# NUS-HPC-AI-Lab/VideoSys

Hardware: AMD Instinct MI355X
Metric: videos/min (Open-Sora 512x512x64f, 30 denoise steps, DiT denoising only) + sec/denoise-step (higher is better)
Workload: dtype bf16; 1 GPU; open-sora-v1.2 STDiT3-XL/2 512x512x64f, latent [4,19,64,64], CFG batch 2 = 38912 token rows, 300 text tokens, depth 28; steps_per_video=30, parallelism=dsp1

## Files before the change

__graft_entry__.py:

```python
from __future__ import annotations

import os
import subprocess
import sys

ROOT = os.path.dirname(os.path.abspath(__file__))
CSRC = os.path.join(ROOT, "videosys_amd", "csrc")
LIB = os.path.join(ROOT, "videosys_amd", "libvideosys_amd.so")
SOURCES = ["gemm_bf16.hip", "gemm2_bf16.hip", "conv_bf16.hip", "vae_ops.hip", "vae_sd3.hip", "vae_osp.hip", "t5_ops.hip", "clip_ops.hip", "rowwise.hip", "adaln_fold.hip", "attention.hip", "attention_w64.hip",
           "attention_t3.hip", "attention64.hip", "attention64_w64.hip", "attention_t64.hip", "attention96.hip", "attention96_img.hip", "p2p.hip", "capi.hip", "program.hip"]
LAB = os.environ.get("VSYS_LAB") == "1"
LAB_SOURCES = ["gemm3_bf16.hip", "gemm4_bf16.hip"]


def _hipcc():
    for c in (os.environ.get("HIPCC"), "/opt/rocm/bin/hipcc", "hipcc"):
        if c and (os.path.isabs(c) and os.path.exists(c) or not os.path.isabs(c)):
            return c
    return "hipcc"


HEADERS = [os.path.join(CSRC, "common.h"), os.path.join(CSRC, "vsys_internal.h"), os.path.join(CSRC, "flash72_w64_asm.inc"),
           os.path.join(CSRC, "program_ops.inc"), os.path.join(CSRC, "flash_w64.h"), os.path.join(CSRC, "attention96.h"), os.path.join(CSRC, "flash72_w64_map.inc"),
           os.path.join(ROOT, "include", "videosys_amd.h"),
           os.path.join(ROOT, "include", "videosys_amd_lab.h")]
FLAGS = ["--offload-arch=gfx950", "-O3", "-std=c++17", "-fPIC"]


def _is_lab(path):
    with open(path, "rb") as fh:
        return b"vsys_lab_flash_debug_buffer" in fh.read()


def _hipcc_id():
    try:
        return subprocess.run([_hipcc(), "--version"], capture_output=True, text=True, timeout=60).stdout.strip()[:400]
    except Exception:
        return "unknown"


def _digest(src, header_blob, flags, cc_id):
    import hashlib

    h = hashlib.sha256()
    h.update(cc_id.encode())
    h.update(" ".join(flags).encode())
    h.update(header_blob)
    with open(src, "rb") as fh:
        h.update(fh.read())
    return h.hexdigest()


ASM_OWNED = {"attention_w64.hip": 224, "attention64_w64.hip": 224}


def audit_asm_register_ownership(src: str, flags=None) -> None:
    import re
    import tempfile

    lo = ASM_OWNED[os.path.basename(src)]
    with tempfile.TemporaryDirectory() as d:
        out = os.path.join(d, "k.s")
        subprocess.run([_hipcc()] + (flags or FLAGS) + ["-S", "--cuda-device-only", "-o", out, src], check=True, capture_output=True,
                       cwd=CSRC)
        text = open(out).read().split("\n")
    inside, bad = False, []
    for ln in text:
        if "#ASMSTART" in ln:
            inside = True
        elif "#ASMEND" in ln:
            inside = False
        elif not inside and not ln.lstrip().startswith((".", ";")):
            code = ln.split(";")[0]
            regs = [int(m) for m in re.findall(r"\ba\[?(\d+)", code)]
            if any(r < lo for r in regs) or ("v_accvgpr" in code and not regs) or "scratch_" in code:
                bad.append(ln.strip())
    if bad:
        raise RuntimeError(f"{os.path.basename(src)}: compiler-generated code touches the asm statements' registers a[0:{lo - 1}] "
                           f"(or spills): {bad[:5]}")


def compile_library(out: str, lab: bool = False, objdir: str = None, force: bool = False) -> bool:
    import json
    from concurrent.futures import ThreadPoolExecutor

    import shutil

    if shutil.which(_hipcc()) is None and not os.path.isabs(_hipcc()) and os.path.exists(out) and not force:
        try:
            import json as _json

            with open(os.path.join(objdir or os.path.join(CSRC, "build", "lab" if lab else "ship"), "manifest.json")) as fh:
                man = _json.load(fh)
            blob = b""
            for h in HEADERS:
                with open(h, "rb") as fh:
                    blob += fh.read()
            flags = FLAGS + (["-DVSYS_LAB"] if lab else [])
            cc_id = man.get("compiler", "unknown")
            srcs = SOURCES + (LAB_SOURCES if lab else [])
            stale = [s_ for s_ in srcs if man.get("objects", {}).get(s_) != _digest(os.path.join(CSRC, s_), blob, flags, cc_id)]
        except Exception as e:
            stale = [f"(manifest unreadable: {e})"]
        if stale:
            raise RuntimeError(f"no hipcc on this box and the shipped {os.path.basename(out)} was not built from the current sources "
# ... 144 lines not shown
```

videosys_amd/csrc/rowwise.hip:

```cpp
#include "common.h"

#include <cstdlib>
#include "vsys_internal.h"

namespace vsys {
namespace {

template <int MAXV>
__global__ __launch_bounds__(256) void adaln_modulate_kernel(const bf16_t* __restrict__ x, const bf16_t* __restrict__ shift,
                                                             const bf16_t* __restrict__ scale, bf16_t* __restrict__ y,
                                                             int64_t rows, int C, int64_t rows_per_sample,
                                                             int64_t mod_stride, float eps) {
  const int lane = threadIdx.x & 63;
  const int64_t row = (int64_t)blockIdx.x * 4 + (threadIdx.x >> 6);
  if (row >= rows) return;
  const int nchunk = C >> 3;
  const bf16_t* xr = x + row * C;
  float v[MAXV][8];
  float s = 0.f;
#pragma unroll
  for (int i = 0; i < MAXV; ++i) {
    const int c = lane + 64 * i;
    if (c < nchunk) {
      uint4 u = *reinterpret_cast<const uint4*>(xr + c * 8);
      unpack8(u, v[i]);
#pragma unroll
      for (int e = 0; e < 8; ++e) s += v[i][e];
    }
  }
  const float mean = wave_sum(s) / (float)C;
  float q = 0.f;
#pragma unroll
  for (int i = 0; i < MAXV; ++i) {
    const int c = lane + 64 * i;
    if (c < nchunk) {
#pragma unroll
      for (int e = 0; e < 8; ++e) {
        float d = v[i][e] - mean;
        q += d * d;
      }
    }
  }
  const float rstd = rsqrtf(wave_sum(q) / (float)C + eps);
  const int64_t b = row / rows_per_sample;
  const bf16_t* sh = shift + b * mod_stride;
  const bf16_t* sc = scale + b * mod_stride;
  bf16_t* yr = y + row * C;
#pragma unroll
  for (int i = 0; i < MAXV; ++i) {
    const int c = lane + 64 * i;
    if (c < nchunk) {
      float a[8], m[8], o[8];
      unpack8(*reinterpret_cast<const uint4*>(sh + c * 8), a);
      unpack8(*reinterpret_cast<const uint4*>(sc + c * 8), m);
#pragma unroll
      for (int e = 0; e < 8; ++e) o[e] = (v[i][e] - mean) * rstd * (1.0f + m[e]) + a[e];
      *reinterpret_cast<uint4*>(yr + c * 8) = pack8(o);
    }
  }
}

template <int RPW>
__global__ __launch_bounds__(256) void adaln_modulate_rows_kernel(const bf16_t* __restrict__ x, const bf16_t* __restrict__ shift,
                                                                  const bf16_t* __restrict__ scale, bf16_t* __restrict__ y,
                                                                  int64_t rows, int C, int64_t rows_per_sample,
                                                                  int64_t mod_stride, float eps) {
  constexpr int MAXV = 3;
  const int lane = threadIdx.x & 63;
  const int64_t row0 = ((int64_t)blockIdx.x * 4 + (threadIdx.x >> 6)) * RPW;
  if (row0 >= rows) return;
  const int nchunk = C >> 3;
  uint4 u[RPW][MAXV];
#pragma unroll
  for (int r = 0; r < RPW; ++r) {
    const int64_t row = row0 + r < rows ? row0 + r : rows - 1;
#pragma unroll
    for (int i = 0; i < MAXV; ++i) {
      const int c = lane + 64 * i;
      u[r][i] = c < nchunk ? *reinterpret_cast<const uint4*>(x + row * C + c * 8) : make_uint4(0, 0, 0, 0);
    }
  }
  const int64_t b = row0 / rows_per_sample;
  uint4 ush[MAXV], usc[MAXV];
#pragma unroll
  for (int i = 0; i < MAXV; ++i) {
    const int c = lane + 64 * i;
    ush[i] = c < nchunk ? *reinterpret_cast<const uint4*>(shift + b * mod_stride + c * 8) : make_uint4(0, 0, 0, 0);
    usc[i] = c < nchunk ? *reinterpret_cast<const uint4*>(scale + b * mod_stride + c * 8) : make_uint4(0, 0, 0, 0);
  }
// ... 89 lines not shown
        float w[8], bb[8];
        unpack8(*reinterpret_cast<const uint4*>(ln_w + c * 8), w);
        unpack8(*reinterpret_cast<const uint4*>(ln_b + c * 8), bb);
#pragma unroll
        for (int e = 0; e < 8; ++e) o[e] = o[e] * w[e] + bb[e];
      }
      if (shift != nullptr) {
        float a[8], m[8];
        unpack8(*reinterpret_cast<const uint4*>(shift + b * mod_stride + alt + c * 8), a);
        unpack8(*reinterpret_cast<const uint4*>(scale + b * mod_stride + alt + c * 8), m);
#pragma unroll
        for (int e = 0; e < 8; ++e) o[e] = o[e] * (1.0f + m[e]) + a[e];
      }
      *reinterpret_cast<uint4*>(yr + c * 8) = pack8(o);
    }
  }
}

__global__ void gate_add_rows_kernel(bf16_t* __restrict__ x, const bf16_t* __restrict__ y, const bf16_t* __restrict__ gate,
                                     int64_t rows, int C8, int64_t rows_per_sample, int64_t gate_stride, int64_t seg_split,
                                     int64_t gate_alt) {
  const int64_t total = rows * C8;
  for (int64_t i = (int64_t)blockIdx.x * blockDim.x + threadIdx.x; i < total; i += (int64_t)gridDim.x * blockDim.x) {
    const int64_t r = i / C8;
    const int c = (int)(i - r * C8);
    const int64_t b = r / rows_per_sample;
    const int64_t alt = (seg_split > 0 && r - b * rows_per_sample < seg_split) ? gate_alt : 0;
    float a[8], v[8], g[8];
    unpack8(reinterpret_cast<const uint4*>(x)[i], a);
    unpack8(reinterpret_cast<const uint4*>(y)[i], v);
    unpack8(*reinterpret_cast<const uint4*>(gate + b * gate_stride + alt + c * 8), g);
#pragma unroll
    for (int k = 0; k < 8; ++k) a[k] += bf2f(f2bf(g[k] * v[k]));
    reinterpret_cast<uint4*>(x)[i] = pack8(a);
  }
}

__global__ void im2col_patch_kernel(const float* __restrict__ z, int Bz, bf16_t* __restrict__ out, int B, int F, int Cin, int H,
                                    int W, int p) {
  const int Hp = H / p, Wp = W / p, K = Cin * p * p;
  const int64_t total = (int64_t)B * F * Hp * Wp * K;
  for (int64_t i = (int64_t)blockIdx.x * blockDim.x + threadIdx.x; i < total; i += (int64_t)gridDim.x * blockDim.x) {
    const int k = (int)(i % K);
    const int64_t tok = i / K;
    const int wp = (int)(tok % Wp), hp = (int)((tok / Wp) % Hp), f = (int)((tok / ((int64_t)Wp * Hp)) % F);
    const int b = (int)(tok / ((int64_t)Wp * Hp * F));
    const int dx = k % p, dy = (k / p) % p, c = k / (p * p);
    out[i] = f2bf(z[((((int64_t)(b % Bz) * F + f) * Cin + c) * H + hp * p + dy) * W + wp * p + dx]);
  }
}

__global__ void unpatchify_cvx_kernel(const bf16_t* __restrict__ x, int64_t ldx, float* __restrict__ out, int B, int F, int Hp,
                                      int Wp, int Cout, int p) {
  const int H = Hp * p, W = Wp * p;
  const int64_t total = (int64_t)B * F * Cout * H * W;
  for (int64_t i = (int64_t)blockIdx.x * blockDim.x + threadIdx.x; i < total; i += (int64_t)gridDim.x * blockDim.x) {
    const int w = (int)(i % W), h = (int)((i / W) % H), c = (int)((i / ((int64_t)W * H)) % Cout);
    const int64_t bf = i / ((int64_t)W * H * Cout);
    const int64_t tok = (bf * Hp + h / p) * Wp + w / p;
    out[i] = bf2f(x[tok * ldx + (c * p + h % p) * p + w % p]);
  }
}

__global__ void mod_table_kernel(const bf16_t* __restrict__ table, const bf16_t* __restrict__ t_mlp, bf16_t* __restrict__ out,
                                 int nblk, int B, int C6) {
  const int64_t i = (int64_t)blockIdx.x * blockDim.x + threadIdx.x;
  const int64_t total = (int64_t)nblk * B * C6;
  if (i >= total) return;
  const int c = (int)(i % C6);
  const int b = (int)((i / C6) % B);
  const int k = (int)(i / ((int64_t)C6 * B));
  out[i] = f2bf(bf2f(table[(int64_t)k * C6 + c]) + bf2f(t_mlp[(int64_t)b * C6 + c]));
}

__global__ void timestep_embedding_kernel(const float* __restrict__ t, bf16_t* __restrict__ out, int B, int dim) {
  const int i = blockIdx.x * blockDim.x + threadIdx.x;
  const int half = dim / 2;
  if (i >= B * half) return;
  const int b = i / half, k = i - b * half;
  const float f = expf(-9.210340371976184f * (float)k / (float)half);
  const float a = t[b] * f;
  out[(int64_t)b * dim + k] = f2bf(cosf(a));
  out[(int64_t)b * dim + half + k] = f2bf(sinf(a));
}

__global__ __launch_bounds__(256) void patch_embed_kernel(const float* __restrict__ x, int Bz, const bf16_t* __restrict__ w,
                                                          const bf16_t* __restrict__ bias, const bf16_t* __restrict__ pos,
                                                          bf16_t* __restrict__ out, int B, int Cin, int T, int H, int W,
                                                          int ph, int pw, int C, int s0, int Sl) {
  const int Hp = (H + ph - 1) / ph, Wp = (W + pw - 1) / pw;
  const int S = Hp * Wp;
  const int cchunks = C >> 3;
  const int64_t total = (int64_t)B * T * Sl * cchunks;
  const int64_t i = (int64_t)blockIdx.x * blockDim.x + threadIdx.x;
  if (i >= total) return;
  const int cc = (int)(i % cchunks);
  const int64_t tok = i / cchunks;
  const int s = s0 + (int)(tok % Sl);
  const int t = (int)((tok / Sl) % T);
  const int b = (int)(tok / ((int64_t)Sl * T));
  const int bz = b % Bz;
  if (s >= S) {
    *reinterpret_cast<uint4*>(out + tok * C + cc * 8) = make_uint4(0, 0, 0, 0);
    return;
  }
  const int hp = s / Wp, wp = s - hp * Wp;
  float acc[8];
  {
    float bb[8];
    unpack8(*reinterpret_cast<const uint4*>(bias + cc * 8), bb);
#pragma unroll
    for (int e = 0; e < 8; ++e) acc[e] = bb[e];
  }
  const int K = Cin * ph * pw;
  if (K == 16) {
    float xin[16];
#pragma unroll
    for (int k = 0; k < 16; ++k) {
      const int ci = k >> 2, dy = (k >> 1) & 1, dx = k & 1;
      const int hh = hp * 2 + dy, ww = wp * 2 + dx;
      xin[k] = 0.f;
      if (ph == 2 && pw == 2 && hh < H && ww < W) xin[k] = bf2f(f2bf(x[((((int64_t)bz * Cin + ci) * T + t) * H + hh) * W + ww]));
    }
    if (ph == 2 && pw == 2) {
#pragma unroll
      for (int e = 0; e < 8; ++e) {
        const bf16_t* wr = w + (int64_t)(cc * 8 + e) * 16;
        float wa[8], wb[8];
        unpack8(*reinterpret_cast<const uint4*>(wr), wa);
        unpack8(*reinterpret_cast<const uint4*>(wr + 8), wb);
#pragma unroll
        for (int k = 0; k < 8; ++k) acc[e] += xin[k] * wa[k] + xin[k + 8] * wb[k];
      }
    }
  }
  if (!(K == 16 && ph == 2 && pw == 2)) {
    for (int ci = 0; ci < Cin; ++ci)
      for (int dy = 0; dy < ph; ++dy)
        for (int dx = 0; dx < pw; ++dx) {
          const int hh = hp * ph + dy, ww = wp * pw + dx;
          float xv = 0.f;
          if (hh < H && ww < W) xv = bf2f(f2bf(x[((((int64_t)bz * Cin + ci) * T + t) * H + hh) * W + ww]));
          const int k = (ci * ph + dy) * pw + dx;
#pragma unroll
          for (int e = 0; e < 8; ++e) acc[e] += xv * bf2f(w[(int64_t)(cc * 8 + e) * K + k]);
        }
  }
  float pp[8];
  unpack8(*reinterpret_cast<const uint4*>(pos + (int64_t)s * C + cc * 8), pp);
#pragma unroll
  for (int e = 0; e < 8; ++e) acc[e] = bf2f(f2bf(acc[e])) + pp[e];
  *reinterpret_cast<uint4*>(out + tok * C + cc * 8) = pack8(acc);
}

template <int MAXV>
__global__ __launch_bounds__(256) void final_layer_kernel(const bf16_t* __restrict__ x, const bf16_t* __restrict__ table,
                                                          const bf16_t* __restrict__ tvec, const bf16_t* __restrict__ w,
                                                          const bf16_t* __restrict__ bias, float* __restrict__ out,
                                                          int B, int T, int Hp, int Wp, int H, int W, int ph, int pw,
                                                          int Cout, int C, float eps, int Sl, float* __restrict__ tokens) {
  const int lane = threadIdx.x & 63;
  const int S = Sl;
  const int64_t rows = (int64_t)B * T * S;
  const int64_t row = (int64_t)blockIdx.x * 4 + (threadIdx.x >> 6);
  if (row >= rows) return;
  const int nchunk = C >> 3;
  const bf16_t* xr = x + row * C;
  float v[MAXV][8];
  float s = 0.f;
#pragma unroll
  for (int i = 0; i < MAXV; ++i) {
    const int c = lane + 64 * i;
    if (c < nchunk) {
      unpack8(*reinterpret_cast<const uint4*>(xr + c * 8), v[i]);
#pragma unroll
      for (int e = 0; e < 8; ++e) s += v[i][e];
    } else {
#pragma unroll
      for (int e = 0; e < 8; ++e) v[i][e] = 0.f;
    }
  }
  const float mean = wave_sum(s) / (float)C;
  float q = 0.f;
#pragma unroll
  for (int i = 0; i < MAXV; ++i) {
    const int c = lane + 64 * i;
    if (c < nchunk) {
#pragma unroll
      for (int e = 0; e < 8; ++e) {
        float d = v[i][e] - mean;
        q += d * d;
      }
    }
  }
  const float rstd = rsqrtf(wave_sum(q) / (float)C + eps);
  const int b = (int)(row / ((int64_t)T * S));
#pragma unroll
  for (int i = 0; i < MAXV; ++i) {
    const int c = lane + 64 * i;
    if (c < nchunk) {
      float sh[8], sc[8], tt[8];
      unpack8(*reinterpret_cast<const uint4*>(table + c * 8), sh);
      unpack8(*reinterpret_cast<const uint4*>(table + C + c * 8), sc);
      unpack8(*reinterpret_cast<const uint4*>(tvec + (int64_t)b * C + c * 8), tt);
#pragma unroll
      for (int e = 0; e < 8; ++e) {
        const float shift = bf2f(f2bf(sh[e] + tt[e])), scale = bf2f(f2bf(sc[e] + tt[e]));
        v[i][e] = bf2f(f2bf((v[i][e] - mean) * rstd * (1.0f + scale) + shift));
      }
    }
  }
  const int NOUT = ph * pw * Cout;
  const int64_t tok = row % ((int64_t)T * S);
  const int t = (int)(tok / S), sidx = (int)(tok % S);
  const int hp = sidx / Wp, wp = sidx - hp * Wp;
  for (int n = 0; n < NOUT; ++n) {
    const bf16_t* wr = w + (int64_t)n * C;
    float d = 0.f;
#pragma unroll
    for (int i = 0; i < MAXV; ++i) {
      const int c = lane + 64 * i;
      if (c < nchunk) {
        float ww[8];
        unpack8(*reinterpret_cast<const uint4*>(wr + c * 8), ww);
#pragma unroll
        for (int e = 0; e < 8; ++e) d += v[i][e] * ww[e];
      }
    }
    d = wave_sum(d);
    if (lane == 0) {
      d = bf2f(f2bf(d + bf2f(bias[n])));
      if (tokens != nullptr) {
        tokens[row * NOUT + n] = d;
        continue;
      }
      const int co = n % Cout;
      const int dx = (n / Cout) % pw, dy = n / (Cout * pw);
      const int hh = hp * ph + dy, ww2 = wp * pw + dx;
      if (hh < H && ww2 < W) out[((((int64_t)b * Cout + co) * T + t) * H + hh) * W + ww2] = d;
    }
  }
}

__global__ void unpatchify_tokens_kernel(const float* __restrict__ tok, float* __restrict__ out, int P, int B, int T, int Sl,
                                         int Hp, int Wp, int H, int W, int ph, int pw, int Cout) {
  const int NOUT = ph * pw * Cout;
  const int64_t total = (int64_t)B * Cout * T * H * W;
  const int64_t i = (int64_t)blockIdx.x * blockDim.x + threadIdx.x;
  if (i >= total) return;
  const int ww = (int)(i % W), hh = (int)((i / W) % H), t = (int)((i / ((int64_t)W * H)) % T);
  const int co = (int)((i / ((int64_t)W * H * T)) % Cout), b = (int)(i / ((int64_t)W * H * T * Cout));
  const int hp = hh / ph, dy = hh - hp * ph, wp = ww / pw, dx = ww - wp * pw;
  const int s = hp * Wp + wp;
  const int r = s / Sl, j = s - r * Sl;
  const int n = (dy * pw + dx) * Cout + co;
  out[i] = tok[((((int64_t)r * B + b) * T + t) * Sl + j) * NOUT + n];
}

__global__ void cfg_euler_kernel(float* __restrict__ z, const float* __restrict__ model_out, int Bz, int Cin, int Cout,
                                 int64_t thw, float guidance, float dt) {
  const int64_t i = (int64_t)blockIdx.x * blockDim.x + threadIdx.x;
  const int64_t total = (int64_t)Bz * Cin * thw;
  if (i >= total) return;
  const int64_t sp = i % thw;
  const int c = (int)((i / thw) % Cin);
  const int b = (int)(i / (thw * Cin));
  const float cond = model_out[((int64_t)b * Cout + c) * thw + sp];
  const float unc = model_out[((int64_t)(b + Bz) * Cout + c) * thw + sp];
  z[i] = z[i] + (unc + guidance * (cond - unc)) * dt;
}

__global__ void cfg_axpby_kernel(float* __restrict__ z, const float* __restrict__ model_out, int Bz, int Cin, int Cout,
                                 int64_t thw, float guidance, float c_z, float c_eps, int cond_first) {
  const int64_t i = (int64_t)blockIdx.x * blockDim.x + threadIdx.x;
  const int64_t total = (int64_t)Bz * Cin * thw;
  if (i >= total) return;
  const int64_t sp = i % thw;
  const int c = (int)((i / thw) % Cin);
  const int b = (int)(i / (thw * Cin));
  const float h0 = model_out[((int64_t)b * Cout + c) * thw + sp];
  const float h1 = model_out[((int64_t)(b + Bz) * Cout + c) * thw + sp];
  const float cond = cond_first ? h0 : h1, unc = cond_first ? h1 : h0;
  z[i] = c_z * z[i] + c_eps * (unc + guidance * (cond - unc));
}

__global__ void add_bcast_rows_kernel(bf16_t* __restrict__ x, const bf16_t* __restrict__ e, int64_t rows, int C8, int64_t group,
                                      int64_t period) {
  const int64_t total = rows * C8;
  for (int64_t i = (int64_t)blockIdx.x * blockDim.x + threadIdx.x; i < total; i += (int64_t)gridDim.x * blockDim.x) {
    const int64_t r = i / C8;
    const int c = (int)(i - r * C8);
    const int64_t er = (r / group) % period;
    float a[8], b[8];
    unpack8(reinterpret_cast<const uint4*>(x)[i], a);
    unpack8(reinterpret_cast<const uint4*>(e)[er * C8 + c], b);
#pragma unroll
    for (int k = 0; k < 8; ++k) a[k] += b[k];
    reinterpret_cast<uint4*>(x)[i] = pack8(a);
  }
}

__global__ void add_rows_kernel(bf16_t* __restrict__ x, const bf16_t* __restrict__ y, int64_t n8) {
  for (int64_t i = (int64_t)blockIdx.x * blockDim.x + threadIdx.x; i < n8; i += (int64_t)gridDim.x * blockDim.x) {
    float a[8], b[8];
    unpack8(reinterpret_cast<const uint4*>(x)[i], a);
    unpack8(reinterpret_cast<const uint4*>(y)[i], b);
#pragma unroll
    for (int e = 0; e < 8; ++e) a[e] += b[e];
    reinterpret_cast<uint4*>(x)[i] = pack8(a);
  }
}

__global__ void scale_add_rows_kernel(const bf16_t* __restrict__ a, int64_t lda, const bf16_t* __restrict__ b, int64_t ldb,
                                      bf16_t* __restrict__ out, int64_t ldo, int64_t rows, int C8, float scale) {
  const int64_t total = rows * C8;
  for (int64_t i = (int64_t)blockIdx.x * blockDim.x + threadIdx.x; i < total; i += (int64_t)gridDim.x * blockDim.x) {
    const int64_t r = i / C8;
    const int c = (int)(i - r * C8) * 8;
    float x[8], y[8];
    unpack8(*reinterpret_cast<const uint4*>(a + r * lda + c), x);
    unpack8(*reinterpret_cast<const uint4*>(b + r * ldb + c), y);
#pragma unroll
// ... 78 lines not shown
    hipLaunchKernelGGL(adaln_modulate_kernel<2>, dim3(grid), dim3(256), 0, stream, x, shift, scale, y, rows, C,
                       rows_per_sample, mod_stride, eps);
  else if (C <= 64 * 8 * 3)
    hipLaunchKernelGGL(adaln_modulate_kernel<3>, dim3(grid), dim3(256), 0, stream, x, shift, scale, y, rows, C,
                       rows_per_sample, mod_stride, eps);
  else
    hipLaunchKernelGGL(adaln_modulate_kernel<4>, dim3(grid), dim3(256), 0, stream, x, shift, scale, y, rows, C,
                       rows_per_sample, mod_stride, eps);
  return hipGetLastError() == hipSuccess ? 0 : VSYS_ERR_LAUNCH;
}

int launch_ln_modulate(const bf16_t* x, const bf16_t* ln_w, const bf16_t* ln_b, const bf16_t* shift, const bf16_t* scale,
                       bf16_t* y, int64_t rows, int C, int64_t rows_per_sample, int64_t mod_stride, int64_t seg_split,
                       int64_t mod_alt, float eps, hipStream_t stream) {
  if (rows <= 0) return 0;
  if (C % 8 != 0 || C > 64 * 8 * 6 || rows_per_sample <= 0 || (mod_stride % 8) || (mod_alt % 8)) return VSYS_ERR_SHAPE;
  if ((ln_w == nullptr) != (ln_b == nullptr) || (shift == nullptr) != (scale == nullptr)) return VSYS_ERR_ARG;
  const unsigned grid = (unsigned)((rows + 3) / 4);
#define VSYS_LNMOD(V)                                                                                                      \
  hipLaunchKernelGGL(ln_modulate_kernel<V>, dim3(grid), dim3(256), 0, stream, x, ln_w, ln_b, shift, scale, y, rows, C,       \
                     rows_per_sample, mod_stride, seg_split, mod_alt, eps)
  if (C <= 64 * 8 * 2) VSYS_LNMOD(2);
  else if (C <= 64 * 8 * 3) VSYS_LNMOD(3);
  else if (C <= 64 * 8 * 4) VSYS_LNMOD(4);
  else VSYS_LNMOD(6);
#undef VSYS_LNMOD
  return hipGetLastError() == hipSuccess ? 0 : VSYS_ERR_LAUNCH;
}

int launch_gate_add_rows(bf16_t* x, const bf16_t* y, const bf16_t* gate, int64_t rows, int C, int64_t rows_per_sample,
                         int64_t gate_stride, int64_t seg_split, int64_t gate_alt, hipStream_t stream) {
  if (rows <= 0) return 0;
  if (C % 8 || rows_per_sample <= 0 || (gate_stride % 8) || (gate_alt % 8)) return VSYS_ERR_SHAPE;
  int64_t grid = (rows * (C / 8) + 255) / 256;
  if (grid > 2048 * 4) grid = 2048 * 4;
  hipLaunchKernelGGL(gate_add_rows_kernel, dim3((unsigned)grid), dim3(256), 0, stream, x, y, gate, rows, C / 8, rows_per_sample,
                     gate_stride, seg_split, gate_alt);
  return hipGetLastError() == hipSuccess ? 0 : VSYS_ERR_LAUNCH;
}

int launch_im2col_patch(const float* z, int Bz, bf16_t* out, int B, int F, int Cin, int H, int W, int p, hipStream_t stream) {
  if (p <= 0 || H % p || W % p || Bz <= 0) return VSYS_ERR_SHAPE;
  const int64_t total = (int64_t)B * F * (H / p) * (W / p) * Cin * p * p;
  if (total <= 0) return 0;
  int64_t grid = (total + 255) / 256;
  if (grid > 2048 * 8) grid = 2048 * 8;
  hipLaunchKernelGGL(im2col_patch_kernel, dim3((unsigned)grid), dim3(256), 0, stream, z, Bz, out, B, F, Cin, H, W, p);
  return hipGetLastError() == hipSuccess ? 0 : VSYS_ERR_LAUNCH;
}

int launch_unpatchify_cvx(const bf16_t* x, int64_t ldx, float* out, int B, int F, int Hp, int Wp, int Cout, int p,
                          hipStream_t stream) {
  const int64_t total = (int64_t)B * F * Cout * Hp * p * Wp * p;
  if (total <= 0) return 0;
  int64_t grid = (total + 255) / 256;
  if (grid > 2048 * 8) grid = 2048 * 8;
  hipLaunchKernelGGL(unpatchify_cvx_kernel, dim3((unsigned)grid), dim3(256), 0, stream, x, ldx, out, B, F, Hp, Wp, Cout, p);
  return hipGetLastError() == hipSuccess ? 0 : VSYS_ERR_LAUNCH;
}

int launch_mod_table(const bf16_t* table, const bf16_t* t_mlp, bf16_t* out, int nblk, int B, int C6, hipStream_t stream) {
  const int64_t total = (int64_t)nblk * B * C6;
  if (total <= 0) return 0;
  hipLaunchKernelGGL(mod_table_kernel, dim3((unsigned)((total + 255) / 256)), dim3(256), 0, stream, table, t_mlp, out, nblk,
                     B, C6);
  return hipGetLastError() == hipSuccess ? 0 : VSYS_ERR_LAUNCH;
}

int launch_timestep_embedding(const float* t, bf16_t* out, int B, int dim, hipStream_t stream) {
  if (dim % 2) return VSYS_ERR_SHAPE;
  const int total = B * (dim / 2);
  if (total <= 0) return 0;
  hipLaunchKernelGGL(timestep_embedding_kernel, dim3((total + 127) / 128), dim3(128), 0, stream, t, out, B, dim);
  return hipGetLastError() == hipSuccess ? 0 : VSYS_ERR_LAUNCH;
}

int launch_patch_embed(const float* x, int Bz, const bf16_t* w, const bf16_t* bias, const bf16_t* pos, bf16_t* out, int B,
                       int Cin, int T, int H, int W, int ph, int pw, int C, int s0, int Sl, hipStream_t stream) {
  if (C % 8 || Bz <= 0 || s0 < 0) return VSYS_ERR_SHAPE;
  const int Hp = (H + ph - 1) / ph, Wp = (W + pw - 1) / pw;
  if (Sl < 0) Sl = Hp * Wp;
  const int64_t total = (int64_t)B * T * Sl * (C / 8);
  if (total <= 0) return 0;
  if ((total + 255) / 256 > 0x7fffffff) return VSYS_ERR_SHAPE;
  hipLaunchKernelGGL(patch_embed_kernel, dim3((unsigned)((total + 255) / 256)), dim3(256), 0, stream, x, Bz, w, bias, pos, out,
                     B, Cin, T, H, W, ph, pw, C, s0, Sl);
  return hipGetLastError() == hipSuccess ? 0 : VSYS_ERR_LAUNCH;
}

int launch_unpatchify_tokens(const float* tok, float* out, int P, int B, int T, int Sl, int Hp, int Wp, int H, int W, int ph,
                             int pw, int Cout, hipStream_t stream) {
  if (P <= 0 || Sl <= 0 || (int64_t)P * Sl < (int64_t)Hp * Wp) return VSYS_ERR_SHAPE;
  const int64_t total = (int64_t)B * Cout * T * H * W;
  if (total <= 0) return 0;
  if ((total + 255) / 256 > 0x7fffffff) return VSYS_ERR_SHAPE;
  hipLaunchKernelGGL(unpatchify_tokens_kernel, dim3((unsigned)((total + 255) / 256)), dim3(256), 0, stream, tok, out, P, B, T, Sl,
                     Hp, Wp, H, W, ph, pw, Cout);
  return hipGetLastError() == hipSuccess ? 0 : VSYS_ERR_LAUNCH;
}

int launch_final_layer(const bf16_t* x, const bf16_t* table, const bf16_t* tvec, const bf16_t* w, const bf16_t* bias,
                       float* out, int B, int T, int Hp, int Wp, int H, int W, int ph, int pw, int Cout, int C, float eps,
                       int Sl, float* tokens, hipStream_t stream) {
  if (C % 8 != 0 || C > 64 * 8 * 4) return VSYS_ERR_SHAPE;
  if (Sl < 0) Sl = Hp * Wp;
  if (tokens == nullptr && Sl != Hp * Wp) return VSYS_ERR_ARG;
  const int64_t rows = (int64_t)B * T * Sl;
  if (rows <= 0) return 0;
  const unsigned grid = (unsigned)((rows + 3) / 4);
  if (C <= 64 * 8 * 2)
    hipLaunchKernelGGL(final_layer_kernel<2>, dim3(grid), dim3(256), 0, stream, x, table, tvec, w, bias, out, B, T, Hp, Wp,
                       H, W, ph, pw, Cout, C, eps, Sl, tokens);
  else if (C <= 64 * 8 * 3)
    hipLaunchKernelGGL(final_layer_kernel<3>, dim3(grid), dim3(256), 0, stream, x, table, tvec, w, bias, out, B, T, Hp, Wp,
                       H, W, ph, pw, Cout, C, eps, Sl, tokens);
  else
    hipLaunchKernelGGL(final_layer_kernel<4>, dim3(grid), dim3(256), 0, stream, x, table, tvec, w, bias, out, B, T, Hp, Wp,
                       H, W, ph, pw, Cout, C, eps, Sl, tokens);
  return hipGetLastError() == hipSuccess ? 0 : VSYS_ERR_LAUNCH;
}

int launch_cfg_euler(float* z, const float* model_out, int Bz, int Cin, int Cout, int64_t thw, float guidance, float dt,
                     hipStream_t stream) {
  const int64_t total = (int64_t)Bz * Cin * thw;
  if (total <= 0) return 0;
  hipLaunchKernelGGL(cfg_euler_kernel, dim3((unsigned)((total + 255) / 256)), dim3(256), 0, stream, z, model_out, Bz, Cin,
                     Cout, thw, guidance, dt);
  return hipGetLastError() == hipSuccess ? 0 : VSYS_ERR_LAUNCH;
}

int launch_cfg_axpby(float* z, const float* model_out, int Bz, int Cin, int Cout, int64_t thw, float guidance, float c_z,
                     float c_eps, int cond_first, hipStream_t stream) {
  const int64_t total = (int64_t)Bz * Cin * thw;
  if (total <= 0) return 0;
  hipLaunchKernelGGL(cfg_axpby_kernel, dim3((unsigned)((total + 255) / 256)), dim3(256), 0, stream, z, model_out, Bz, Cin,
                     Cout, thw, guidance, c_z, c_eps, cond_first);
  return hipGetLastError() == hipSuccess ? 0 : VSYS_ERR_LAUNCH;
}

int launch_add_bcast_rows(bf16_t* x, const bf16_t* e, int64_t rows, int C, int64_t group, int64_t period, hipStream_t stream) {
  if (rows <= 0) return 0;
  if (C % 8 || group <= 0 || period <= 0) return VSYS_ERR_SHAPE;
  int64_t grid = (rows * (C / 8) + 255) / 256;
  if (grid > 2048 * 4) grid = 2048 * 4;
  hipLaunchKernelGGL(add_bcast_rows_kernel, dim3((unsigned)grid), dim3(256), 0, stream, x, e, rows, C / 8, group, period);
  return hipGetLastError() == hipSuccess ? 0 : VSYS_ERR_LAUNCH;
}

int launch_add_rows(bf16_t* x, const bf16_t* y, int64_t n, hipStream_t stream) {
  if (n <= 0) return 0;
  if (n % 8) return VSYS_ERR_SHAPE;
  const int64_t n8 = n / 8;
  int64_t grid = (n8 + 255) / 256;
  if (grid > 2048 * 4) grid = 2048 * 4;
  hipLaunchKernelGGL(add_rows_kernel, dim3((unsigned)grid), dim3(256), 0, stream, x, y, n8);
  return hipGetLastError() == hipSuccess ? 0 : VSYS_ERR_LAUNCH;
}

int launch_scale_add_rows(const bf16_t* a, int64_t lda, const bf16_t* b, int64_t ldb, bf16_t* out, int64_t ldo, int64_t rows, int C,
                          float scale, hipStream_t stream) {
  if (rows < 0 || C < 0) return VSYS_ERR_SHAPE;
  if (rows == 0 || C == 0) return 0;
  if (C % 8 || lda < C || ldb < C || ldo < C) return VSYS_ERR_SHAPE;
  if ((lda % 8) || (ldb % 8) || (ldo % 8) || reinterpret_cast<uintptr_t>(a) % 16 || reinterpret_cast<uintptr_t>(b) % 16 ||
      reinterpret_cast<uintptr_t>(out) % 16)
    return VSYS_ERR_ALIGN;
  int64_t grid = (rows * (C / 8) + 255) / 256;
  if (grid > 2048 * 4) grid = 2048 * 4;
  hipLaunchKernelGGL(scale_add_rows_kernel, dim3((unsigned)grid), dim3(256), 0, stream, a, lda, b, ldb, out, ldo, rows, C / 8, scale);
  return hipGetLastError() == hipSuccess ? 0 : VSYS_ERR_LAUNCH;
}

int launch_copy_4d(const bf16_t* src, bf16_t* dst, int n0, int n1, int n2, int C, int64_t ss0, int64_t ss1, int64_t ss2,
                   int64_t ds0, int64_t ds1, int64_t ds2, int n1_valid, int n2_valid, hipStream_t stream) {
  if (C % 8) return VSYS_ERR_SHAPE;
  const int64_t total = (int64_t)n0 * n1 * n2 * (C / 8);
  if (total <= 0) return 0;
  int64_t grid = (total + 255) / 256;
  if (grid > 2048 * 4) grid = 2048 * 4;
  hipLaunchKernelGGL(copy_4d_kernel, dim3((unsigned)grid), dim3(256), 0, stream, src, dst, n0, n1, n2, C, ss0, ss1, ss2, ds0,
                     ds1, ds2, n1_valid, n2_valid);
  return hipGetLastError() == hipSuccess ? 0 : VSYS_ERR_LAUNCH;
}

}
```

Before: 21.32 videos/min.

## Add persistent tiled kernels for patch embedding and final layer

```diff
diff --git a/__graft_entry__.py b/__graft_entry__.py
--- a/__graft_entry__.py
+++ b/__graft_entry__.py
@@ -20,7 +20,7 @@
     return "hipcc"
 
 
-HEADERS = [os.path.join(CSRC, "common.h"), os.path.join(CSRC, "vsys_internal.h"), os.path.join(CSRC, "flash72_w64_asm.inc"),
+HEADERS = [os.path.join(CSRC, "common.h"), os.path.join(CSRC, "vsys_internal.h"), os.path.join(CSRC, "rowwise_plan.h"), os.path.join(CSRC, "flash72_w64_asm.inc"),
            os.path.join(CSRC, "program_ops.inc"), os.path.join(CSRC, "flash_w64.h"), os.path.join(CSRC, "attention96.h"), os.path.join(CSRC, "flash72_w64_map.inc"),
            os.path.join(ROOT, "include", "videosys_amd.h"),
            os.path.join(ROOT, "include", "videosys_amd_lab.h")]
diff --git a/videosys_amd/csrc/rowwise.hip b/videosys_amd/csrc/rowwise.hip
--- a/videosys_amd/csrc/rowwise.hip
+++ b/videosys_amd/csrc/rowwise.hip
@@ -2,9 +2,15 @@
 
 #include <cstdlib>
 #include "vsys_internal.h"
+#include "rowwise_plan.h"
 
 namespace vsys {
 namespace {
+
+bool rowwise_edges_on() {
+  static const bool on = [] { const char* e = getenv("VSYS_ROWWISE_EDGES"); return !(e && e[0] == '0'); }();
+  return on;
+}
 
 template <int MAXV>
 __global__ __launch_bounds__(256) void adaln_modulate_kernel(const bf16_t* __restrict__ x, const bf16_t* __restrict__ shift,
@@ -260,6 +266,35 @@
   const float a = t[b] * f;
   out[(int64_t)b * dim + k] = f2bf(cosf(a));
   out[(int64_t)b * dim + half + k] = f2bf(sinf(a));
+}
+
+__device__ __forceinline__ void pe_bias_init(float (&acc)[8], const uint4& bias8) {
+  float bb[8];
+  unpack8(bias8, bb);
+#pragma unroll
+  for (int e = 0; e < 8; ++e) acc[e] = bb[e];
+}
+__device__ __forceinline__ void pe_load_weights(const bf16_t* __restrict__ w, int cc, float (&wa)[8][8], float (&wb)[8][8]) {
+#pragma unroll
+  for (int e = 0; e < 8; ++e) {
+    const bf16_t* wr = w + (int64_t)(cc * 8 + e) * 16;
+    unpack8(*reinterpret_cast<const uint4*>(wr), wa[e]);
+    unpack8(*reinterpret_cast<const uint4*>(wr + 8), wb[e]);
+  }
+}
+__device__ __forceinline__ void pe_conv16(float (&acc)[8], const float (&xin)[16], const float (&wa)[8][8], const float (&wb)[8][8]) {
+#pragma unroll
+  for (int e = 0; e < 8; ++e) {
+#pragma unroll
+    for (int k = 0; k < 8; ++k) acc[e] += xin[k] * wa[e][k] + xin[k + 8] * wb[e][k];
+  }
+}
+__device__ __forceinline__ uint4 pe_finish(float (&acc)[8], const uint4& pos8) {
+  float pp[8];
+  unpack8(pos8, pp);
+#pragma unroll
+  for (int e = 0; e < 8; ++e) acc[e] = bf2f(f2bf(acc[e])) + pp[e];
+  return pack8(acc);
 }
 
 __global__ __launch_bounds__(256) void patch_embed_kernel(const float* __restrict__ x, int Bz, const bf16_t* __restrict__ w,
@@ -284,12 +319,7 @@
   }
   const int hp = s / Wp, wp = s - hp * Wp;
   float acc[8];
-  {
-    float bb[8];
-    unpack8(*reinterpret_cast<const uint4*>(bias + cc * 8), bb);
-#pragma unroll
-    for (int e = 0; e < 8; ++e) acc[e] = bb[e];
-  }
+  pe_bias_init(acc, *reinterpret_cast<const uint4*>(bias + cc * 8));
   const int K = Cin * ph * pw;
   if (K == 16) {
     float xin[16];
@@ -301,15 +331,9 @@
       if (ph == 2 && pw == 2 && hh < H && ww < W) xin[k] = bf2f(f2bf(x[((((int64_t)bz * Cin + ci) * T + t) * H + hh) * W + ww]));
     }
     if (ph == 2 && pw == 2) {
-#pragma unroll
-      for (int e = 0; e < 8; ++e) {
-        const bf16_t* wr = w + (int64_t)(cc * 8 + e) * 16;
-        float wa[8], wb[8];
-        unpack8(*reinterpret_cast<const uint4*>(wr), wa);
-        unpack8(*reinterpret_cast<const uint4*>(wr + 8), wb);
-#pragma unroll
-        for (int k = 0; k < 8; ++k) acc[e] += xin[k] * wa[k] + xin[k + 8] * wb[k];
-      }
+      float wa[8][8], wb[8][8];
+      pe_load_weights(w, cc, wa, wb);
+      pe_conv16(acc, xin, wa, wb);
     }
   }
   if (!(K == 16 && ph == 2 && pw == 2)) {
@@ -324,12 +348,160 @@
           for (int e = 0; e < 8; ++e) acc[e] += xv * bf2f(w[(int64_t)(cc * 8 + e) * K + k]);
         }
   }
-  float pp[8];
-  unpack8(*reinterpret_cast<const uint4*>(pos + (int64_t)s * C + cc * 8), pp);
-#pragma unroll
-  for (int e = 0; e < 8; ++e) acc[e] = bf2f(f2bf(acc[e])) + pp[e];
-  *reinterpret_cast<uint4*>(out + tok * C + cc * 8) = pack8(acc);
-}
+  *reinterpret_cast<uint4*>(out + tok * C + cc * 8) = pe_finish(acc, *reinterpret_cast<const uint4*>(pos + (int64_t)s * C + cc * 8));
+}
+
+__global__ __launch_bounds__(PE_CHUNK_LANES* PE_TOKEN_LANES) void patch_embed_runs_kernel(
+    const float* __restrict__ x, int Bz, const bf16_t* __restrict__ w, const bf16_t* __restrict__ bias, const bf16_t* __restrict__ pos,
+    bf16_t* __restrict__ out, int B, int T, int H, int W, int C, int s0, int Sl, int runs_per_row, int run_len) {
+  constexpr int Cin = 4, NT = PE_CHUNK_LANES * PE_TOKEN_LANES;
+  __shared__ float xs[2 * Cin][2 * PE_RUN_TOKENS];
+  const int Hp = (H + 1) / 2, Wp = (W + 1) / 2;
+  const int cchunks = C >> 3;
+  const int tid = threadIdx.x;
+  const int tl = tid / PE_CHUNK_LANES;
+  const int cc = blockIdx.y * PE_CHUNK_LANES + (tid - tl * PE_CHUNK_LANES);
+  const bool active = cc < cchunks;
+  float wa[8][8], wb[8][8];
+  uint4 bias8 = make_uint4(0, 0, 0, 0);
+  if (active) {
+    pe_load_weights(w, cc, wa, wb);
+    bias8 = *reinterpret_cast<const uint4*>(bias + cc * 8);
+  }
+  const int hp0 = s0 / Wp, hp1 = (int)(((int64_t)s0 + Sl + Wp - 1) / Wp);
+  const int nhp = hp1 - hp0;
+  const int64_t nruns = (int64_t)B * T * nhp * runs_per_row;
+  for (int64_t run = blockIdx.x; run < nruns; run += gridDim.x) {
+    const int rw = (int)(run % runs_per_row);
+    int64_t r = run / runs_per_row;
+    const int hp = hp0 + (int)(r % nhp);
+    r /= nhp;
+    const int t = (int)(r % T), b = (int)(r / T);
+    const int wp0 = rw * run_len;
+    const int ntok = (Wp - wp0 < run_len ? Wp - wp0 : run_len);
+    if (hp < Hp) {
+      const int bz = b % Bz;
+      const int ncol = 2 * ntok;
+      for (int i = tid; i < 2 * Cin * ncol; i += NT) {
+        const int rr = i / ncol, col = i - rr * ncol;
+        const int hh = hp * 2 + (rr & 1), ww = wp0 * 2 + col;
+        float v = 0.f;
+        if (hh < H && ww < W) v = bf2f(f2bf(x[((((int64_t)bz * Cin + (rr >> 1)) * T + t) * H + hh) * W + ww]));
+        xs[rr][col] = v;
+      }
+    }
+    __syncthreads();
+    if (active) {
+      const int sb = hp * Wp + wp0;
+      auto load_pos = [&](int j) {
+        const int s = sb + j;
+        return (j < ntok && hp < Hp && s >= s0 && s - s0 < Sl) ? *reinterpret_cast<const uint4*>(pos + (int64_t)s * C + cc * 8)
+                                                              : make_uint4(0, 0, 0, 0);
+      };
+      uint4 p0 = load_pos(tl), p1 = load_pos(tl + PE_TOKEN_LANES);
+      for (int j = tl; j < ntok; j += PE_TOKEN_LANES) {
+        const uint4 pos8 = p0;
+        p0 = p1;
+        p1 = load_pos(j + 2 * PE_TOKEN_LANES);
+        const int s = sb + j;
+        if (s >= s0 && s - s0 < Sl) {
+          bf16_t* o = out + (((int64_t)b * T + t) * Sl + (s - s0)) * C + cc * 8;
+          if (hp >= Hp) {
+            *reinterpret_cast<uint4*>(o) = make_uint4(0, 0, 0, 0);
+          } else {
+            float xin[16];
+#pragma unroll
+            for (int q = 0; q < 8; ++q) {
+              const float2 p = *reinterpret_cast<const float2*>(&xs[q][2 * j]);
+              xin[2 * q] = p.x;
+              xin[2 * q + 1] = p.y;
+            }
+            float acc[8];
+            pe_bias_init(acc, bias8);
+            pe_conv16(acc, xin, wa, wb);
+            *reinterpret_cast<uint4*>(o) = pe_finish(acc, pos8);
+          }
+        }
+      }
+    }
+    __syncthreads();
+  }
+}
+
+template <int MAXV>
+__device__ __forceinline__ void fl_load_row(uint4 (&u)[MAXV], const bf16_t* __restrict__ xr, int lane, int nchunk) {
+#pragma unroll
+  for (int i = 0; i < MAXV; ++i) {
+    const int c = lane + 64 * i;
+    u[i] = c < nchunk ? *reinterpret_cast<const uint4*>(xr + c * 8) : make_uint4(0, 0, 0, 0);
+  }
+}
+template <int MAXV>
+__device__ __forceinline__ float fl_row_sum(const uint4 (&u)[MAXV], float (&v)[MAXV][8], int lane, int nchunk) {
+  float s = 0.f;
+#pragma unroll
+  for (int i = 0; i < MAXV; ++i) {
+    const int c = lane + 64 * i;
+    if (c < nchunk) {
+      unpack8(u[i], v[i]);
+#pragma unroll
+      for (int e = 0; e < 8; ++e) s += v[i][e];
+    } else {
+#pragma unroll
+      for (int e = 0; e < 8; ++e) v[i][e] = 0.f;
+    }
+  }
+  return s;
+}
+template <int MAXV>
+__device__ __forceinline__ void fl_row_stats(const float (&v)[MAXV][8], float s, int lane, int nchunk, int C, float eps, float& mean,
+                                             float& rstd) {
+  mean = wave_sum(s) / (float)C;
+  float q = 0.f;
+#pragma unroll
+  for (int i = 0; i < MAXV; ++i) {
+    const int c = lane + 64 * i;
+    if (c < nchunk) {
+#pragma unroll
+      for (int e = 0; e < 8; ++e) {
+        float d = v[i][e] - mean;
+        q += d * d;
+      }
+    }
+  }
+  rstd = rsqrtf(wave_sum(q) / (float)C + eps);
+}
+__device__ __forceinline__ void fl_shift_scale8(const uint4& sh8, const uint4& sc8, const uint4& tt8, float (&shift)[8], float (&scale)[8]) {
+  float sh[8], sc[8], tt[8];
+  unpack8(sh8, sh);
+  unpack8(sc8, sc);
+  unpack8(tt8, tt);
+#pragma unroll
+  for (int e = 0; e < 8; ++e) {
+    shift[e] = bf2f(f2bf(sh[e] + tt[e]));
+    scale[e] = bf2f(f2bf(sc[e] + tt[e]));
+  }
+}
+__device__ __forceinline__ void fl_modulate8(float (&v)[8], float mean, float rstd, const float (&shift)[8], const float (&scale)[8]) {
+#pragma unroll
+  for (int e = 0; e < 8; ++e) v[e] = bf2f(f2bf((v[e] - mean) * rstd * (1.0f + scale[e]) + shift[e]));
+}
+template <int MAXV>
+__device__ __forceinline__ float fl_dot(const float (&v)[MAXV][8], const uint4* wrow, int lane, int nchunk) {
+  float d = 0.f;
+#pragma unroll
+  for (int i = 0; i < MAXV; ++i) {
+    const int c = lane + 64 * i;
+    if (c < nchunk) {
+      float ww[8];
+      unpack8(wrow[c], ww);
+#pragma unroll
+      for (int e = 0; e < 8; ++e) d += v[i][e] * ww[e];
+    }
+  }
+  return d;
+}
+__device__ __forceinline__ float fl_out(float d, bf16_t bias_n) { return bf2f(f2bf(d + bf2f(bias_n))); }
 
 template <int MAXV>
 __global__ __launch_bounds__(256) void final_layer_kernel(const bf16_t* __restrict__ x, const bf16_t* __restrict__ table,
@@ -343,49 +515,21 @@
   const int64_t row = (int64_t)blockIdx.x * 4 + (threadIdx.x >> 6);
   if (row >= rows) return;
   const int nchunk = C >> 3;
-  const bf16_t* xr = x + row * C;
+  uint4 u[MAXV];
+  fl_load_row<MAXV>(u, x + row * C, lane, nchunk);
   float v[MAXV][8];
-  float s = 0.f;
+  const float s = fl_row_sum<MAXV>(u, v, lane, nchunk);
+  float mean, rstd;
+  fl_row_stats<MAXV>(v, s, lane, nchunk, C, eps, mean, rstd);
+  const int b = (int)(row / ((int64_t)T * S));
 #pragma unroll
   for (int i = 0; i < MAXV; ++i) {
     const int c = lane + 64 * i;
     if (c < nchunk) {
-      unpack8(*reinterpret_cast<const uint4*>(xr + c * 8), v[i]);
-#pragma unroll
-      for (int e = 0; e < 8; ++e) s += v[i][e];
-    } else {
-#pragma unroll
-      for (int e = 0; e < 8; ++e) v[i][e] = 0.f;
-    }
-  }
-  const float mean = wave_sum(s) / (float)C;
-  float q = 0.f;
-#pragma unroll
-  for (int i = 0; i < MAXV; ++i) {
-    const int c = lane + 64 * i;
-    if (c < nchunk) {
-#pragma unroll
-      for (int e = 0; e < 8; ++e) {
-        float d = v[i][e] - mean;
-        q += d * d;
-      }
-    }
-  }
-  const float rstd = rsqrtf(wave_sum(q) / (float)C + eps);
-  const int b = (int)(row / ((int64_t)T * S));
-#pragma unroll
-  for (int i = 0; i < MAXV; ++i) {
-    const int c = lane + 64 * i;
-    if (c < nchunk) {
-      float sh[8], sc[8], tt[8];
-      unpack8(*reinterpret_cast<const uint4*>(table + c * 8), sh);
-      unpack8(*reinterpret_cast<const uint4*>(table + C + c * 8), sc);
-      unpack8(*reinterpret_cast<const uint4*>(tvec + (int64_t)b * C + c * 8), tt);
-#pragma unroll
-      for (int e = 0; e < 8; ++e) {
-        const float shift = bf2f(f2bf(sh[e] + tt[e])), scale = bf2f(f2bf(sc[e] + tt[e]));
-        v[i][e] = bf2f(f2bf((v[i][e] - mean) * rstd * (1.0f + scale) + shift));
-      }
+      float shift[8], scale[8];
+      fl_shift_scale8(*reinterpret_cast<const uint4*>(table + c * 8), *reinterpret_cast<const uint4*>(table + C + c * 8),
+                      *reinterpret_cast<const uint4*>(tvec + (int64_t)b * C + c * 8), shift, scale);
+      fl_modulate8(v[i], mean, rstd, shift, scale);
     }
   }
   const int NOUT = ph * pw * Cout;
@@ -393,21 +537,10 @@
   const int t = (int)(tok / S), sidx = (int)(tok % S);
   const int hp = sidx / Wp, wp = sidx - hp * Wp;
   for (int n = 0; n < NOUT; ++n) {
-    const bf16_t* wr = w + (int64_t)n * C;
-    float d = 0.f;
-#pragma unroll
-    for (int i = 0; i < MAXV; ++i) {
-      const int c = lane + 64 * i;
-      if (c < nchunk) {
-        float ww[8];
-        unpack8(*reinterpret_cast<const uint4*>(wr + c * 8), ww);
-#pragma unroll
-        for (int e = 0; e < 8; ++e) d += v[i][e] * ww[e];
-      }
-    }
+    float d = fl_dot<MAXV>(v, reinterpret_cast<const uint4*>(w + (int64_t)n * C), lane, nchunk);
     d = wave_sum(d);
     if (lane == 0) {
-      d = bf2f(f2bf(d + bf2f(bias[n])));
+      d = fl_out(d, bias[n]);
       if (tokens != nullptr) {
         tokens[row * NOUT + n] = d;
         continue;
@@ -416,6 +549,114 @@
       const int dx = (n / Cout) % pw, dy = n / (Cout * pw);
       const int hh = hp * ph + dy, ww2 = wp * pw + dx;
       if (hh < H && ww2 < W) out[((((int64_t)b * Cout + co) * T + t) * H + hh) * W + ww2] = d;
+    }
+  }
+}
+
+template <int MAXV>
+__global__ __launch_bounds__(FL_WAVES * 64, MAXV <= 3 ? 2 : 1) void final_layer_rows_kernel(
+    const bf16_t* __restrict__ x, const bf16_t* __restrict__ table, const bf16_t* __restrict__ tvec, const bf16_t* __restrict__ w,
+    const bf16_t* __restrict__ bias, float* __restrict__ out, int B, int T, int Hp, int Wp, int H, int W, int ph, int pw, int Cout, int C,
+    float eps, int Sl, float* __restrict__ tokens) {
+  extern __shared__ uint4 fl_lds[];
+  constexpr int NT = FL_WAVES * 64;
+  const int tid = threadIdx.x, lane = tid & 63, wave = tid >> 6;
+  const int nchunk = C >> 3;
+  const int NOUT = ph * pw * Cout;
+  const int pitch = NOUT + 1;
+  uint4* wl = fl_lds;
+  float* stage = reinterpret_cast<float*>(fl_lds + NOUT * nchunk);
+  for (int i = tid; i < NOUT * nchunk; i += NT) wl[i] = reinterpret_cast<const uint4*>(w)[i];
+  __syncthreads();
+  const int S = Sl;
+  const int64_t rows = (int64_t)B * T * S;
+  const int64_t ntiles = (rows + FL_TILE_ROWS - 1) / FL_TILE_ROWS;
+  bf16_t bias_bits = 0;
+  if (lane < NOUT) bias_bits = bias[lane];
+  uint4 u[MAXV];
+#pragma unroll
+  for (int i = 0; i < MAXV; ++i) u[i] = make_uint4(0, 0, 0, 0);
+  {
+    const int64_t row = (int64_t)blockIdx.x * FL_TILE_ROWS + wave * FL_ROWS_PER_WAVE;
+    if (row < rows) fl_load_row<MAXV>(u, x + row * C, lane, nchunk);
+  }
+  int cur_b = -1;
+  uint4 shp[MAXV], scp[MAXV];
+  for (int64_t tile = blockIdx.x; tile < ntiles; tile += gridDim.x) {
+#pragma unroll
+    for (int k = 0; k < FL_ROWS_PER_WAVE; ++k) {
+      const int64_t row = tile * FL_TILE_ROWS + wave * FL_ROWS_PER_WAVE + k;
+      const int64_t nrow = k + 1 < FL_ROWS_PER_WAVE ? row + 1 : (tile + gridDim.x) * FL_TILE_ROWS + wave * FL_ROWS_PER_WAVE;
+      uint4 un[MAXV];
+#pragma unroll
+      for (int i = 0; i < MAXV; ++i) un[i] = make_uint4(0, 0, 0, 0);
+      if (nrow < rows) fl_load_row<MAXV>(un, x + nrow * C, lane, nchunk);
+      if (row < rows) {
+        float v[MAXV][8];
+        const float s = fl_row_sum<MAXV>(u, v, lane, nchunk);
+        float mean, rstd;
+        fl_row_stats<MAXV>(v, s, lane, nchunk, C, eps, mean, rstd);
+        const int b = (int)(row / ((int64_t)T * S));
+        if (b != cur_b) {
+          cur_b = b;
+#pragma unroll
+          for (int i = 0; i < MAXV; ++i) {
+            const int c = lane + 64 * i;
+            if (c < nchunk) {
+              float shift[8], scale[8];
+              fl_shift_scale8(*reinterpret_cast<const uint4*>(table + c * 8), *reinterpret_cast<const uint4*>(table + C + c * 8),
+                              *reinterpret_cast<const uint4*>(tvec + (int64_t)b * C + c * 8), shift, scale);
+              shp[i] = pack8(shift);
+              scp[i] = pack8(scale);
+            }
+          }
+        }
+#pragma unroll
+        for (int i = 0; i < MAXV; ++i) {
+          if (lane + 64 * i < nchunk) {
+            float shift[8], scale[8];
+            unpack8(shp[i], shift);
+            unpack8(scp[i], scale);
+            fl_modulate8(v[i], mean, rstd, shift, scale);
+          }
+        }
+        float keep = 0.f;
+        for (int n0 = 0; n0 < NOUT; n0 += 4) {
+#pragma unroll
+          for (int jn = 0; jn < 4; ++jn) {
+            const int n = n0 + jn;
+            float d = fl_dot<MAXV>(v, wl + (n < NOUT ? n : NOUT - 1) * nchunk, lane, nchunk);
+            d = wave_sum(d);
+            keep = lane == n ? d : keep;
+          }
+        }
+        if (lane < NOUT) {
+          const float y = fl_out(keep, bias_bits);
+          if (tokens != nullptr) tokens[row * NOUT + lane] = y;
+          else stage[(wave * FL_ROWS_PER_WAVE + k) * pitch + lane] = y;
+        }
+      }
+#pragma unroll
+      for (int i = 0; i < MAXV; ++i) u[i] = un[i];
+    }
+    if (tokens == nullptr) {
+      __syncthreads();
+      const int per = FL_TILE_ROWS * pw;
+      for (int j = tid; j < FL_TILE_ROWS * NOUT; j += NT) {
+        const int g = j / per, rem = j - g * per;
+        const int r = rem / pw, dx = rem - r * pw;
+        const int co = g / ph, dy = g - co * ph;
+        const int64_t row = tile * FL_TILE_ROWS + r;
+        if (row >= rows) continue;
+        const int n = (dy * pw + dx) * Cout + co;
+        const int b = (int)(row / ((int64_t)T * S));
+        const int64_t tok = row % ((int64_t)T * S);
+        const int t = (int)(tok / S), sidx = (int)(tok % S);
+        const int hp = sidx / Wp, wp = sidx - hp * Wp;
+        const int hh = hp * ph + dy, ww2 = wp * pw + dx;
+        if (hh < H && ww2 < W) out[((((int64_t)b * Cout + co) * T + t) * H + hh) * W + ww2] = stage[r * pitch + n];
+      }
+      __syncthreads();
     }
   }
 }
@@ -660,6 +901,17 @@
   if (Sl < 0) Sl = Hp * Wp;
   const int64_t total = (int64_t)B * T * Sl * (C / 8);
   if (total <= 0) return 0;
+  if (rowwise_edges_on() && patch_embed_runs_ok(Cin, ph, pw, C) && Wp > 0) {
+    const int runs_per_row = patch_embed_runs_per_row(Wp), run_len = patch_embed_run_len(Wp);
+    const int64_t nhp = ((int64_t)s0 + Sl + Wp - 1) / Wp - s0 / Wp;
+    const int64_t nruns = (int64_t)B * T * nhp * runs_per_row;
+    const int64_t most = cu_count_this_device();
+    const unsigned gx = (unsigned)(nruns < most ? nruns : most);
+    const unsigned gy = (unsigned)((C / 8 + PE_CHUNK_LANES - 1) / PE_CHUNK_LANES);
+    hipLaunchKernelGGL(patch_embed_runs_kernel, dim3(gx, gy), dim3(PE_CHUNK_LANES * PE_TOKEN_LANES), 0, stream, x, Bz, w, bias, pos, out,
+                       B, T, H, W, C, s0, Sl, runs_per_row, run_len);
+    return hipGetLastError() == hipSuccess ? 0 : VSYS_ERR_LAUNCH;
+  }
   if ((total + 255) / 256 > 0x7fffffff) return VSYS_ERR_SHAPE;
   hipLaunchKernelGGL(patch_embed_kernel, dim3((unsigned)((total + 255) / 256)), dim3(256), 0, stream, x, Bz, w, bias, pos, out,
                      B, Cin, T, H, W, ph, pw, C, s0, Sl);
@@ -685,6 +937,28 @@
   if (tokens == nullptr && Sl != Hp * Wp) return VSYS_ERR_ARG;
   const int64_t rows = (int64_t)B * T * Sl;
   if (rows <= 0) return 0;
+  const int lds = rowwise_edges_on() ? final_layer_rows_lds(ph * pw * Cout, C) : 0;
+  if (lds > 0) {
+    static std::atomic<unsigned long long> seen{0};
+    for (DeviceOnce once(seen); once.todo(); once.done()) {
+      (void)hipFuncSetAttribute((const void*)final_layer_rows_kernel<2>, hipFuncAttributeMaxDynamicSharedMemorySize, ROWWISE_LDS_BUDGET);
+      (void)hipFuncSetAttribute((const void*)final_layer_rows_kernel<3>, hipFuncAttributeMaxDynamicSharedMemorySize, ROWWISE_LDS_BUDGET);
+      (void)hipFuncSetAttribute((const void*)final_layer_rows_kernel<4>, hipFuncAttributeMaxDynamicSharedMemorySize, ROWWISE_LDS_BUDGET);
+    }
+    const int64_t ntiles = (rows + FL_TILE_ROWS - 1) / FL_TILE_ROWS;
+    const int64_t most = (int64_t)final_layer_rows_per_cu(lds) * cu_count_this_device();
+    const dim3 grid((unsigned)(ntiles < most ? ntiles : most)), block(FL_WAVES * 64);
+    if (C <= 64 * 8 * 2)
+      hipLaunchKernelGGL(final_layer_rows_kernel<2>, grid, block, lds, stream, x, table, tvec, w, bias, out, B, T, Hp, Wp, H, W, ph, pw,
+                         Cout, C, eps, Sl, tokens);
+    else if (C <= 64 * 8 * 3)
+      hipLaunchKernelGGL(final_layer_rows_kernel<3>, grid, block, lds, stream, x, table, tvec, w, bias, out, B, T, Hp, Wp, H, W, ph, pw,
+                         Cout, C, eps, Sl, tokens);
+    else
+      hipLaunchKernelGGL(final_layer_rows_kernel<4>, grid, block, lds, stream, x, table, tvec, w, bias, out, B, T, Hp, Wp, H, W, ph, pw,
+                         Cout, C, eps, Sl, tokens);
+    return hipGetLastError() == hipSuccess ? 0 : VSYS_ERR_LAUNCH;
+  }
   const unsigned grid = (unsigned)((rows + 3) / 4);
   if (C <= 64 * 8 * 2)
     hipLaunchKernelGGL(final_layer_kernel<2>, dim3(grid), dim3(256), 0, stream, x, table, tvec, w, bias, out, B, T, Hp, Wp,
diff --git a/videosys_amd/csrc/rowwise_plan.h b/videosys_amd/csrc/rowwise_plan.h
--- /dev/null
+++ b/videosys_amd/csrc/rowwise_plan.h
@@ -0,0 +1,29 @@
+#pragma once
+
+namespace vsys {
+
+constexpr int ROWWISE_LDS_BUDGET = 160 * 1024;
+
+constexpr int PE_CHUNK_LANES = 144, PE_TOKEN_LANES = 3, PE_RUN_TOKENS = 64;
+constexpr int FL_WAVES = 8, FL_ROWS_PER_WAVE = 2, FL_TILE_ROWS = FL_WAVES * FL_ROWS_PER_WAVE;
+
+inline int patch_embed_runs_ok(int Cin, int ph, int pw, int C) { return Cin == 4 && ph == 2 && pw == 2 && C > 0 && C % 8 == 0; }
+
+inline int patch_embed_runs_per_row(int Wp) { return (Wp + PE_RUN_TOKENS - 1) / PE_RUN_TOKENS; }
+inline int patch_embed_run_len(int Wp) {
+  const int n = patch_embed_runs_per_row(Wp);
+  return n > 0 ? (Wp + n - 1) / n : 0;
+}
+
+inline int final_layer_rows_lds(int nout, int C) {
+  if (nout <= 0 || nout > 64 || C <= 0 || C % 8 != 0) return 0;
+  const long long bytes = (long long)nout * C * 2 + (long long)FL_TILE_ROWS * (nout + 1) * 4;
+  return bytes <= ROWWISE_LDS_BUDGET ? (int)bytes : 0;
+}
+inline int final_layer_rows_per_cu(int lds_bytes) {
+  if (lds_bytes <= 0) return 0;
+  const int n = ROWWISE_LDS_BUDGET / lds_bytes;
+  return n > 2 ? 2 : n;
+}
+
+}
```

Result: no change. 21.45 videos/min (median of 6 runs) (+0.6%).
